# gau-nernst/centernet-lightning

Hardware: AMD Instinct MI355X
Metric: images/sec @512x512 ResNet34 CenterNet forward + gather_detection2d (higher is better)
Workload: dtype f32; 1 GPU; BASELINE C1: ResNet34 + simple neck, 32 img/GPU x 512x512, heads 80+4 (w256), k=100, nms 3; global_batch=32, per_gpu_batch=32, parallelism=batch-shard x1

## Files before the change

### centernet-lightning_amd/centernet_lightning_amd/_lib.py

```python
import ctypes
import os
from ctypes import (POINTER, Structure, c_char_p, c_double, c_float, c_int32, c_int64, c_size_t, c_uint32, c_void_p)

_LIB_NAME = "libcenternet_gfx950.so"
_LIB_PATH = os.path.join(os.path.dirname(os.path.abspath(__file__)), "lib", _LIB_NAME)

CNL_RELU = 1 << 0
CNL_SIGMOID = 1 << 1
CNL_UPSAMPLE_IN = 1 << 2
CNL_UPSAMPLE_OUT_ADD = 1 << 3
CNL_RELU6 = 1 << 4
CNL_W_SPLIT = 1 << 5

CNL_ALGO_AUTO, CNL_ALGO_F2, CNL_ALGO_F32, CNL_ALGO_LATENCY, CNL_ALGO_F43, CNL_ALGO_FORCE = 0, 1, 2, 4, 5, 100
CNL_WINO_F32, CNL_WINO_F16X2 = 2, 5

CNL_E_BAD_ARG, CNL_E_UNSUPPORTED, CNL_E_WORKSPACE, CNL_E_HIP = -1, -2, -3, -4
ABI_VERSION = 13


class ConvParams(Structure):
    _fields_ = [("x", c_void_p), ("w", c_void_p), ("bias", c_void_p), ("residual", c_void_p), ("y", c_void_p),
                ("N", c_int32), ("H_in", c_int32), ("W_in", c_int32), ("Cin", c_int32), ("Cout", c_int32),
                ("KH", c_int32), ("KW", c_int32), ("stride", c_int32), ("pad", c_int32),
# ... 44 lines not shown


class MotTables(Structure):
    POINTERS = ("gt_boxes", "pr_boxes", "gt_ids", "pr_ids", "gt_off", "pr_off", "sim_off", "frm_seq", "seq_frm", "seq_gid", "seq_tid", "seq_pair",
                "seq_idm", "gt_count", "pr_count")
    SCALARS = ("F", "S", "n_gt", "n_pr", "sim_total", "pair_total", "sum_g", "sum_t", "id_total", "max_gids", "max_gt_frame", "max_pr_frame",
               "max_frame_pairs")
    _fields_ = [(n, c_void_p) for n in POINTERS] + [(n, c_int64) for n in SCALARS]


class LossParams(Structure):
    _fields_ = [("stride", c_double), ("target_param", c_double), ("hm_alpha", c_double), ("hm_beta", c_double),
                ("heatmap_weight", c_double), ("box_weight", c_double), ("box_multiplier", c_float), ("target_method", c_int32),
                ("heatmap_loss", c_int32), ("box_loss", c_int32), ("box_log", c_int32), ("reserved", c_int32)]


class ReidLossParams(Structure):
    _fields_ = [("stride", c_double), ("bn_eps", c_double), ("momentum", c_double), ("ignore_index", c_int64), ("center", c_int32),
                ("padded_rows", c_int32), ("training", c_int32), ("reserved", c_int32)]


class AugmentPlacement(Structure):
    _fields_ = [("frame", c_int32), ("x0", c_int32), ("y0", c_int32), ("w", c_int32), ("h", c_int32), ("dx0", c_int32), ("dy0", c_int32),
                ("dw", c_int32), ("dh", c_int32), ("flip", c_int32), ("colour", c_int32 * 12), ("reserved", c_int32 * 2)]


class WarpPlacement(Structure):
    _fields_ = [("frame", c_int32), ("x0", c_int32), ("y0", c_int32), ("w", c_int32), ("h", c_int32), ("dx0", c_int32), ("dy0", c_int32),
                ("dw", c_int32), ("dh", c_int32), ("reserved0", c_int32), ("colour", c_int32 * 12), ("inv", c_int64 * 6), ("fwd", c_double * 6),
                ("reserved", c_int32 * 2)]


assert ctypes.sizeof(LetterboxFrame) == 40 and ctypes.sizeof(AugmentPlacement) == 96 and ctypes.sizeof(WarpPlacement) == 192

_REID_COMMON = [c_void_p, c_int64, c_int64, c_int64, c_int64, c_int32, c_int32, c_int32, c_int32, c_void_p, c_void_p, c_void_p, c_int32,
                c_void_p, c_void_p, c_void_p, c_void_p, c_void_p, c_void_p, c_void_p, c_int32, POINTER(ReidLossParams)]

_SIGNATURES = {
    "cnl_version": (ctypes.c_int, []),
    "cnl_sizeof_params": (c_size_t, [ctypes.c_int32]),
    "cnl_absmax_stride": (ctypes.c_int, []),
    "cnl_last_error": (c_size_t, [c_char_p, c_size_t]),
    "cnl_conv2d_nhwc_f32": (ctypes.c_int, [POINTER(ConvParams), c_void_p]),
    "cnl_fused_out_pack_weights_f32": (ctypes.c_int, [c_void_p, c_void_p, ctypes.c_int32, ctypes.c_int32, c_void_p]),
    "cnl_fused_out_reduce_f32": (ctypes.c_int, [c_void_p, ctypes.c_int32, ctypes.c_int64, ctypes.c_int32, c_void_p, c_void_p, ctypes.c_int32, ctypes.c_uint32, c_void_p]),
    "cnl_pointwise_nhwc_f32": (ctypes.c_int, [POINTER(ConvParams), c_void_p, c_int32, c_int32, c_int32, c_int32, c_int32, c_void_p, c_void_p]),
    "cnl_conv2d_out_hw": (ctypes.c_int, [POINTER(ConvParams), POINTER(c_int32), POINTER(c_int32)]),
    "cnl_conv3x3_winograd_f32": (ctypes.c_int, [POINTER(ConvParams), c_void_p]),
    "cnl_conv3x3_winograd_kernel": (ctypes.c_int, [POINTER(ConvParams)]),
    "cnl_winograd_up_weight_floats": (c_size_t, [ctypes.c_int32, ctypes.c_int32]),
    "cnl_winograd_transform_weights_up_f32": (ctypes.c_int, [c_void_p, c_void_p, ctypes.c_int32, ctypes.c_int32, c_void_p]),
    "cnl_conv3x3_winograd_variant": (ctypes.c_int, [POINTER(ConvParams)]),
    "cnl_conv2d_kernel": (ctypes.c_int, [POINTER(ConvParams)]),
    "cnl_up2_weight_floats": (c_size_t, [ctypes.c_int32, ctypes.c_int32]),
    "cnl_up2_pack_weights_f32": (ctypes.c_int, [c_void_p, c_void_p, ctypes.c_int32, ctypes.c_int32, c_void_p]),
    "cnl_conv3x3_up2_nhwc_f32": (ctypes.c_int, [POINTER(ConvParams), c_void_p]),
    "cnl_conv3x3_up2_kernel": (ctypes.c_int, [POINTER(ConvParams)]),
    "cnl_absmax_per_image_f32": (ctypes.c_int, [c_void_p, ctypes.c_int32, ctypes.c_int64, ctypes.c_int32, ctypes.c_int32, c_void_p, c_void_p]),
    "cnl_winograd_weight_floats": (c_size_t, [c_int32, c_int32]),
    "cnl_winograd_transform_weights_f32": (ctypes.c_int, [c_void_p, c_void_p, c_int32, c_int32, c_void_p]),
    "cnl_deconv2x_nhwc_f32": (ctypes.c_int, [POINTER(DeconvParams), c_void_p]),
    "cnl_deconv_phase_geometry": (ctypes.c_int, [c_int32, c_int32, POINTER(c_int32), POINTER(c_int32)]),
    "cnl_deconv_weight_floats": (c_size_t, [c_int32, c_int32, c_int32]),
    "cnl_conv2d_splitk_scratch_bytes": (c_size_t, [POINTER(ConvParams)]),
    "cnl_fuse_sum_nhwc_f32": (ctypes.c_int, [c_void_p, c_void_p, c_void_p, c_void_p, c_int32, c_int32, c_int32, c_int32, c_int32, c_int32,
                                             c_int32, c_int32, ctypes.c_float, ctypes.c_float, ctypes.c_float, ctypes.c_float, c_int32, c_void_p]),
    "cnl_upsample2x_nhwc_f32": (ctypes.c_int, [c_void_p, c_void_p, c_void_p, c_int32, c_int32, c_int32, c_int32, c_int32, c_int32,
                                               c_int32, c_int32, c_void_p]),
    "cnl_depthwise3x3_nhwc_f32": (ctypes.c_int, [c_void_p, c_void_p, c_void_p, c_void_p, c_int32, c_int32, c_int32, c_int32, c_int32,
                                                 c_int32, c_uint32, c_void_p]),
    "cnl_deform_sample_nhwc_f32": (ctypes.c_int, [c_void_p, c_void_p, c_void_p, c_int32, c_int32, c_int32, c_int32, c_int32, c_int32,
                                                  c_int32, c_int32, c_void_p]),
    "cnl_normalize_u8_nhwc_f32": (ctypes.c_int, [c_void_p, c_void_p, c_int32, c_int32, c_int32, POINTER(c_float), POINTER(c_float), c_void_p]),
    "cnl_resize_bilinear_u8": (ctypes.c_int, [c_void_p, c_void_p, c_int32, c_int32, c_int32, c_int32, c_int32, c_int32, c_void_p]),
    "cnl_letterbox_bilinear_u8": (ctypes.c_int, [c_void_p, c_void_p, c_int32, c_int32, c_int32, c_int32, c_uint32, c_void_p]),
    "cnl_letterbox_yuv420_u8": (ctypes.c_int, [c_void_p, c_void_p, c_int32, c_int32, c_int32, POINTER(c_int32), c_uint32, c_void_p]),
    "cnl_unletterbox_boxes_f32": (ctypes.c_int, [c_void_p, c_void_p, c_int32, c_int32, c_int32, c_void_p]),
    "cnl_crop_boxes_u8": (ctypes.c_int, [c_void_p, c_void_p, c_void_p, c_float, c_void_p, c_int32, c_int32, c_int32, POINTER(c_int32), c_float,
                                         c_int32, c_void_p, c_void_p, c_void_p, c_int32, c_int32, c_uint32, c_void_p]),
    "cnl_draw_boxes_u8": (ctypes.c_int, [c_void_p, c_void_p, c_void_p, c_void_p, c_void_p, c_float, c_void_p, c_int32, c_int32, c_int32, c_int32,
                                         c_void_p, c_int32, c_int32, c_int32, c_int32, c_int32, c_int32, c_void_p, c_void_p]),
    "cnl_flip_merge_f32": (ctypes.c_int, [POINTER(FlipMap), c_int32, c_int32, c_int32, c_int32, c_void_p]),
    "cnl_mirror_append_u8": (ctypes.c_int, [c_void_p, c_void_p, c_int32, c_int32, c_int32, c_int32, c_void_p]),
    "cnl_merge_tiles_workspace_bytes": (c_size_t, [c_int32, c_int32, c_int32, c_int32]),
    "cnl_merge_tiles_f32": (ctypes.c_int, [c_void_p, c_void_p, c_void_p, c_void_p, c_void_p, c_int32, c_int32, c_int32, c_int32, c_int32,
                                           c_float, c_float, c_int32, c_int32, c_void_p, c_void_p, c_void_p, c_void_p, c_void_p, c_void_p,
                                           c_size_t, c_void_p]),
    "cnl_coco_match_f64": (ctypes.c_int, [c_void_p, c_void_p, c_void_p, c_void_p, c_void_p, c_void_p, c_void_p, c_int32, c_int32, c_int32, c_int32,
                                          c_void_p, c_void_p, c_void_p, c_void_p, c_void_p]),
    "cnl_coco_accumulate_f64": (ctypes.c_int, [c_void_p, c_void_p, c_void_p, c_void_p, c_void_p, c_int64, c_int32, c_void_p, c_void_p, c_void_p]),
    "cnl_mot_similarity_f64": (ctypes.c_int, [POINTER(MotTables), c_void_p, c_void_p]),
    "cnl_mot_hota_workspace_bytes": (c_int64, [POINTER(MotTables)]),
    "cnl_mot_hota_f64": (ctypes.c_int, [POINTER(MotTables), c_void_p, c_void_p, c_void_p, c_void_p, c_void_p, c_void_p, c_int64, c_void_p]),
    "cnl_mot_clear_workspace_bytes": (c_int64, [POINTER(MotTables)]),
    "cnl_mot_clear_f64": (ctypes.c_int, [POINTER(MotTables), c_void_p, c_void_p, c_void_p, c_void_p, c_void_p, c_int64, c_void_p]),
    "cnl_mot_identity_workspace_bytes": (c_int64, [POINTER(MotTables)]),
    "cnl_mot_identity_f64": (ctypes.c_int, [POINTER(MotTables), c_void_p, c_void_p, c_void_p, c_void_p, c_void_p, c_int64, c_void_p]),
    "cnl_detection_loss_workspace_bytes": (c_size_t, [c_int32, c_int32, c_int32, c_int32]),
    "cnl_detection_loss_f64": (ctypes.c_int, [c_void_p, c_int64, c_int64, c_int64, c_int64, c_void_p, c_int64, c_int64, c_int64, c_int64,
                                              c_int32, c_int32, c_int32, c_int32, c_void_p, c_void_p, c_void_p, c_int32, POINTER(LossParams),
                                              c_void_p, c_int64, c_int64, c_int64, c_int64, c_void_p, c_void_p, c_void_p, c_void_p, c_size_t,
                                              c_void_p]),
    "cnl_detection_loss_grad_workspace_bytes": (c_size_t, [c_int32, c_int32, c_int32, c_int32]),
    "cnl_detection_loss_grad_f32": (ctypes.c_int, [c_void_p, c_int64, c_int64, c_int64, c_int64, c_void_p, c_int64, c_int64, c_int64, c_int64,
                                                   c_int32, c_int32, c_int32, c_int32, c_void_p, c_void_p, c_void_p, c_int32, POINTER(LossParams),
                                                   c_void_p, c_void_p, c_int64, c_int64, c_int64, c_int64, c_void_p, c_int64, c_int64, c_int64,
# ... 135 lines not shown
```

### centernet-lightning_amd/csrc/conv_args.h

```cpp
#pragma once
#include "cnl_device.h"

namespace cnl_conv {
using namespace cnl_dev;


struct ConvArgs {
    const float* x;
    const float* w;
    const float* bias;
    const float* res;
    float* y;
    int N, Hin, Win, Cin, Cout;
    int KH, KW, stride, pad, pad_x;
    int sub_dy, sub_dx;
    int ldx, ldy, ldr;
    int HL, WL;
    int Ho, Wo, M;
    int CC, KT, K;
    unsigned x_bytes, w_bytes, y_bytes, r_bytes;
    unsigned flags;
    int tiles_n, tiles;
    unsigned mg_hw, sh_hw, mg_w, sh_w;
    long long* trace;
    const float* xmax;
    const float* wmax;
    unsigned* ymax;
    unsigned algo;
    const float* wscale;
    const float* wsplit = nullptr;
    int ksplit = 0, kt_per = 0;
    float* part = nullptr;
    unsigned part_bytes = 0;
};

constexpr unsigned CNL_I_SUBPIXEL = 1u << 16;

template <int WM, int WN, int TM, int TN>
struct Cfg {
    static constexpr int NW = WM * WN;
    static constexpr int THREADS = NW * 64;
    static constexpr int BM = WM * TM * 32;
    static constexpr int BN = WN * TN * 32;
    static constexpr int A_INSTR = BM / (NW * 8);
    static constexpr int B_INSTR = BN / (NW * 8);
    static constexpr int STAGE_BYTES = (BM + BN) * 128;
    static constexpr int LDS_BYTES = 2 * STAGE_BYTES;
    static_assert(NW == 4, "kernel is declared __launch_bounds__(256, 2)");
    static_assert(BM % (NW * 8) == 0 && BN % (NW * 8) == 0, "tile rows must split evenly over waves");
};


__device__ __forceinline__ f32x4 buf_load4(const float* base, unsigned bytes, unsigned voffset, unsigned soffset) {
    const auto rsrc = __builtin_amdgcn_make_buffer_rsrc((void*)base, 0, (int)bytes, 0x00020000);
    return __builtin_bit_cast(f32x4, __builtin_amdgcn_raw_buffer_load_b128(rsrc, voffset, soffset, 0));
}
__device__ __forceinline__ void buf_store4(f32x4 v, float* base, unsigned bytes, unsigned voffset, unsigned soffset) {
    typedef unsigned u32x4_ __attribute__((ext_vector_type(4)));
    const auto rsrc = __builtin_amdgcn_make_buffer_rsrc((void*)base, 0, (int)bytes, 0x00020000);
    __builtin_amdgcn_raw_buffer_store_b128(__builtin_bit_cast(u32x4_, v), rsrc, voffset, soffset, CNL_NT_STORES);
}
__device__ __forceinline__ f32x4 lds_read16(const char* p) { return *reinterpret_cast<const f32x4*>(p); }
__device__ __forceinline__ unsigned fast_div(unsigned n, unsigned magic, unsigned shift) {
    return shift == 0xFFu ? n : (__umulhi(n, magic) >> shift);
}


bool f16x2_eligible(const ConvArgs& a);
int f16x2_launch(const ConvArgs& a, hipStream_t stream);

}
```

### centernet-lightning_amd/csrc/conv_f16x2.hip

```cpp
#include "conv_args.h"
#include <cstdlib>

namespace cnl_conv {



template <int WM, int WN, int TM, int TN, int KS, bool SUB, bool SPLIT = false, bool PREB = false>
__global__ __launch_bounds__(256, 2) void conv_f16x2_kernel(const ConvArgs a) {
    using C = Cfg<WM, WN, TM, TN>;
    constexpr bool PRE = SUB || PREB;
    extern __shared__ __attribute__((aligned(16))) char smem[];
    float* sInv = reinterpret_cast<float*>(smem + C::LDS_BYTES);
    float* sScl = sInv + C::BM;
    int* sImg = reinterpret_cast<int*>(sScl + C::BM);
    unsigned* sPix = reinterpret_cast<unsigned*>(sImg + C::BM);

    const int lane = threadIdx.x & 63;
    const int wave = __builtin_amdgcn_readfirstlane(threadIdx.x >> 6);
    const int wm = wave / WN, wn = wave % WN;
    const int hi = lane >> 5;

    unsigned tile = cnl::xcd_remap(blockIdx.x, (unsigned)a.tiles);
    int slice = 0;
    if constexpr (SPLIT) { slice = (int)(tile % (unsigned)a.ksplit); tile /= (unsigned)a.ksplit; }
    const int kt0 = SPLIT ? slice * a.kt_per : 0;
    const int KTs = SPLIT ? min(a.kt_per, a.KT - kt0) : a.KT;
    const int n_tile = tile % a.tiles_n;
    const int m_tile = tile / a.tiles_n;
    const int m0 = m_tile * C::BM;
    const int n0 = n_tile * C::BN;

    const int lrow = lane >> 3;
    const int pslot = lane & 7;
    unsigned a_mask[C::A_INSTR], a_base[C::A_INSTR];
#pragma unroll
    for (int j = 0; j < C::A_INSTR; ++j) {
        const int r = (j * C::NW + wave) * 8 + lrow;
        const int m = m0 + r;
        const int q = (pslot ^ ((r >> 1) & 7)) * 4;
        const unsigned n = fast_div((unsigned)m, a.mg_hw, a.sh_hw);
        const unsigned rem = (unsigned)m - n * (unsigned)(a.Ho * a.Wo);
        const unsigned oy = fast_div(rem, a.mg_w, a.sh_w);
        const unsigned ox = rem - oy * (unsigned)a.Wo;
        const int iy0 = (int)oy * a.stride - a.pad;
        const int ix0 = (int)ox * a.stride - a.pad_x;
        unsigned mask = 0, xb = 0;
#pragma unroll
        for (int kx = 0; kx < KS; ++kx) xb |= ((unsigned)(ix0 + kx) < (unsigned)a.WL) ? (1u << kx) : 0u;
#pragma unroll
        for (int ky = 0; ky < KS; ++ky) mask |= ((unsigned)(iy0 + ky) < (unsigned)a.HL) ? (xb << (ky * KS)) : 0u;
        a_mask[j] = m < a.M ? mask : 0u;
        const int pix = (int)n * a.Hin * a.Win;
        a_base[j] = (unsigned)(((pix + iy0 * a.Win + ix0) * a.ldx + q) * 4);
    }
    unsigned b_off[C::B_INSTR];
#pragma unroll
    for (int j = 0; j < C::B_INSTR; ++j) {
        const int r = (j * C::NW + wave) * 8 + lrow;
        const int q = (pslot ^ ((r >> 1) & 7)) * 4;
        b_off[j] = (unsigned)(((n0 + r) * a.K + q) * 4);
    }
    unsigned a_voff[C::A_INSTR];
#define C5_TAP(tap_, ky_, kx_)                                                                                    \
    do {                                                                                                          \
        const unsigned bit_ = 1u << (tap_);                                                                       \
        const unsigned delta_ = (unsigned)((((ky_) * a.Win + (kx_)) * a.ldx) * 4);                                \
        _Pragma("unroll") for (int j = 0; j < C::A_INSTR; ++j) a_voff[j] = (a_mask[j] & bit_) ? a_base[j] + delta_ : OOB; \
    } while (0)
// ... 36 lines not shown
            const unsigned oy = fast_div(rem, a.mg_w, a.sh_w);
            const unsigned ox = rem - oy * (unsigned)a.Wo;
            sPix[r] = (n * 2u * (unsigned)a.Ho + 2u * oy + (unsigned)a.sub_dy) * (2u * (unsigned)a.Wo) + 2u * ox + (unsigned)a.sub_dx;
        }
    }

    f32x16 acc[TM][TN];
#pragma unroll
    for (int i = 0; i < TM; ++i)
#pragma unroll
        for (int j = 0; j < TN; ++j) acc[i][j] = mfma_zero();

    const int swz = (lane >> 1) & 7;
    const int a_row_byte = (wm * TM * 32 + (lane & 31)) * 128;
    const int b_row_byte = C::BM * 128 + (wn * TN * 32 + (lane & 31)) * 128;
    f32x4 ra[2][TM], rb[2][TN];
    u32x4 ah[TM], al[TM], bh[TN], bl[TN];
    float sA[TM];

#define C5_READ(stage_ptr_, g_)                                                                                   \
    do {                                                                                                          \
        _Pragma("unroll") for (int q_ = 0; q_ < 2; ++q_) {                                                        \
            const int sb_ = (((2 * (2 * (g_) + q_) + hi) ^ swz) << 4);                                            \
               \
            const int sbb_ = PRE ? (((2 * (2 * (g_) + hi) + q_) ^ swz) << 4) : sb_;                               \
            _Pragma("unroll") for (int i = 0; i < TM; ++i) ra[q_][i] = lds_read16((stage_ptr_) + a_row_byte + i * 32 * 128 + sb_); \
            _Pragma("unroll") for (int j = 0; j < TN; ++j) rb[q_][j] = lds_read16((stage_ptr_) + b_row_byte + j * 32 * 128 + sbb_); \
        }                                                                                                         \
    } while (0)
#define C5_SPLIT()                                                                                                \
    do {                                                                                                          \
        _Pragma("unroll") for (int i = 0; i < TM; ++i) split8(ra[0][i], ra[1][i], sA[i], ah[i], al[i]);           \
        _Pragma("unroll") for (int j = 0; j < TN; ++j) {                                                          \
            if constexpr (PRE) {                                                                                  \
                bh[j] = __builtin_bit_cast(u32x4, rb[0][j]);                                                      \
                bl[j] = __builtin_bit_cast(u32x4, rb[1][j]);                                                      \
            } else {                                                                                              \
                split8(rb[0][j], rb[1][j], Sw, bh[j], bl[j]);                                                     \
            }                                                                                                     \
        }                                                                                                         \
    } while (0)
#define C5_MFMA()                                                                                                 \
    do {                                                                                                          \
        _Pragma("unroll") for (int i = 0; i < TM; ++i)                                                            \
            _Pragma("unroll") for (int j = 0; j < TN; ++j) acc[i][j] = mfma16(ah[i], bl[j], acc[i][j]);           \
        _Pragma("unroll") for (int i = 0; i < TM; ++i)                                                            \
            _Pragma("unroll") for (int j = 0; j < TN; ++j) acc[i][j] = mfma16(al[i], bh[j], acc[i][j]);           \
        _Pragma("unroll") for (int i = 0; i < TM; ++i)                                                            \
            _Pragma("unroll") for (int j = 0; j < TN; ++j) acc[i][j] = mfma16(ah[i], bh[j], acc[i][j]);           \
    } while (0)

    asm volatile("s_waitcnt vmcnt(0)" ::: "memory");
    __syncthreads();
#pragma unroll
    for (int i = 0; i < TM; ++i) sA[i] = sScl[(wm * TM + i) * 32 + (lane & 31)];
    if (KTs > 1) {
        C5_ADVANCE();
        C5_ISSUE(1, cc * 32, (kt0 + 1) * 32);
    }
    C5_READ(smem, 0);
    for (int kt = 0; kt < KTs; ++kt) {
        const char* sS = smem + (kt & 1) * C::STAGE_BYTES;
        const char* sN = smem + ((kt + 1) & 1) * C::STAGE_BYTES;
        C5_SPLIT();
        C5_READ(sS, 1);
        C5_MFMA();
        C5_SPLIT();
        if (kt + 1 < KTs) {
            asm volatile("s_waitcnt vmcnt(0)" ::: "memory");
            __syncthreads();
            if (kt + 2 < KTs) {
                C5_ADVANCE();
                C5_ISSUE(kt & 1, cc * 32, (kt0 + kt + 2) * 32);
            }
            C5_READ(sN, 0);
        }
        C5_MFMA();
    }
#undef C5_TAP
#undef C5_ISSUE
#undef C5_ADVANCE
#undef C5_READ
#undef C5_SPLIT
#undef C5_MFMA

    if constexpr (SPLIT) {
#pragma unroll
        for (int j = 0; j < TN; ++j) {
            const int col = n0 + (wn * TN + j) * 32 + (lane & 31);
#pragma unroll
            for (int i = 0; i < TM; ++i) {
                const int rl = (wm * TM + i) * 32 + 4 * hi;
                const int mb = m0 + rl;
#pragma unroll
                for (int r = 0; r < 16; ++r) {
                    const int ro = (r & 3) + 8 * (r >> 2);
                    const bool ok = col < a.Cout && mb + ro < a.M;
                    buf_store(acc[i][j][r] * sInv[rl + ro], a.part, a.part_bytes,
                              ok ? (unsigned)((((long long)slice * a.M + mb + ro) * a.Cout + col) * 4) : OOB, 0u);
                }
            }
        }
        return;
    }
    const float lo = (a.flags & (CNL_RELU | CNL_RELU6)) ? 0.f : -__builtin_inff();
    const float hi6 = (a.flags & CNL_RELU6) ? 6.f : __builtin_inff();
    const bool sigm = a.flags & CNL_SIGMOID;
    const int img0 = sImg[0];
    float omax = 0.f, omax1 = 0.f;
#pragma unroll
    for (int j = 0; j < TN; ++j) {
        const int col = n0 + (wn * TN + j) * 32 + (lane & 31);
        const bool col_ok = col < a.Cout;
        const float bv = col_ok ? a.bias[col] : 0.f;
#pragma unroll
        for (int i = 0; i < TM; ++i) {
            const int rl = (wm * TM + i) * 32 + 4 * hi;
            const int mb = m0 + rl;
            const unsigned y_voff = (unsigned)((mb * a.ldy + col) * 4);
            const unsigned r_voff = (unsigned)((mb * a.ldr + col) * 4);
            float v[16];
            bool ok[16];
#pragma unroll
            for (int r = 0; r < 16; ++r) {
                const int ro = (r & 3) + 8 * (r >> 2);
                ok[r] = col_ok && mb + ro < a.M;
                v[r] = acc[i][j][r] * sInv[rl + ro] + bv;
            }
            if (!SUB && a.res) {
                float rv[16];
#pragma unroll
                for (int r = 0; r < 16; ++r)
                    rv[r] = buf_load(a.res, a.r_bytes, ok[r] ? r_voff : OOB, (unsigned)(((r & 3) + 8 * (r >> 2)) * a.ldr * 4));
#pragma unroll
                for (int r = 0; r < 16; ++r) v[r] += rv[r];
            }
#pragma unroll
            for (int r = 0; r < 16; ++r) v[r] = fminf(fmaxf(v[r], lo), hi6);
            if (sigm) {
#pragma unroll
                for (int r = 0; r < 16; ++r) v[r] = cnl::fast_sigmoid(v[r]);
            }
            if constexpr (SUB) {
#pragma unroll
                for (int r = 0; r < 16; ++r)
                    buf_store(v[r], a.y, a.y_bytes, ok[r] ? (sPix[rl + (r & 3) + 8 * (r >> 2)] * (unsigned)a.ldy + (unsigned)col) * 4u : OOB, 0u);
            } else {
#pragma unroll
                for (int r = 0; r < 16; ++r)
                    buf_store(v[r], a.y, a.y_bytes, ok[r] ? y_voff : OOB, (unsigned)(((r & 3) + 8 * (r >> 2)) * a.ldy * 4));
            }
            if (a.ymax) {
#pragma unroll
                for (int r = 0; r < 16; ++r) {
                    const float av = ok[r] ? fabsf(v[r]) : 0.f;
                    const int img = sImg[rl + (r & 3) + 8 * (r >> 2)];
                    if (img == img0) omax = fmaxf(omax, av);
                    else if (img == img0 + 1) omax1 = fmaxf(omax1, av);
                    else if (av > 0.f) cnl::report_max(a.ymax + img * AMS, av);
                }
            }
        }
    }
    if (a.ymax) {
#pragma unroll
        for (int o = 32; o > 0; o >>= 1) {
            omax = fmaxf(omax, __shfl_xor(omax, o, 64));
            omax1 = fmaxf(omax1, __shfl_xor(omax1, o, 64));
        }
        if (lane == 0) cnl::report_max(a.ymax + img0 * AMS, omax);
        if (lane == 0) cnl::report_max(a.ymax + (img0 + 1) * AMS, omax1);
    }
}

__global__ __launch_bounds__(256) void splitk_reduce_kernel(const ConvArgs a) {
    const int C4 = (a.Cout + 3) / 4;
    const long total = (long)a.M * C4;
    const long t = (long)blockIdx.x * 256 + threadIdx.x;
    float omax = 0.f;
    int img = -1;
    if (t < total) {
        const int m = (int)(t / C4), col = (int)(t - (long)m * C4) * 4;
        img = (int)fast_div((unsigned)m, a.mg_hw, a.sh_hw);
        const bool vec = col + 4 <= a.Cout && (a.Cout & 3) == 0;
        float v[4] = {0.f, 0.f, 0.f, 0.f};
        const long sstride = (long)a.M * a.Cout;
        const float* p0 = a.part + (long)m * a.Cout + col;
        if (vec) {
            for (int s0 = 0; s0 < a.ksplit; s0 += 8) {
                f32x4 q[8];
#pragma unroll
                for (int j = 0; j < 8; ++j)
                    q[j] = s0 + j < a.ksplit ? *reinterpret_cast<const f32x4*>(p0 + (s0 + j) * sstride) : f32x4{0.f, 0.f, 0.f, 0.f};
#pragma unroll
                for (int j = 0; j < 8; ++j)
#pragma unroll
                    for (int i = 0; i < 4; ++i) v[i] += q[j][i];
            }
        } else {
            for (int s = 0; s < a.ksplit; ++s)
#pragma unroll
                for (int i = 0; i < 4; ++i)
                    if (col + i < a.Cout) v[i] += p0[s * sstride + i];
        }
        const float lo = (a.flags & (CNL_RELU | CNL_RELU6)) ? 0.f : -__builtin_inff();
        const float hi6 = (a.flags & CNL_RELU6) ? 6.f : __builtin_inff();
#pragma unroll
        for (int i = 0; i < 4; ++i) {
            if (col + i >= a.Cout) continue;
            float o = v[i] + a.bias[col + i];
            if (a.res) o += a.res[(long)m * a.ldr + col + i];
            o = fminf(fmaxf(o, lo), hi6);
            if (a.flags & CNL_SIGMOID) o = cnl::fast_sigmoid(o);
            a.y[(long)m * a.ldy + col + i] = o;
            omax = fmaxf(omax, fabsf(o));
        }
    }
    if (a.ymax) {
        const int img0 = __shfl(img, 0, 64);
        const bool same = __all(img == img0 || img < 0);
        if (same) {
#pragma unroll
            for (int o = 32; o > 0; o >>= 1) omax = fmaxf(omax, __shfl_xor(omax, o, 64));
            if ((threadIdx.x & 63) == 0 && img0 >= 0) cnl::report_max(a.ymax + img0 * AMS, omax);
        } else if (img >= 0 && omax > 0.f) {
            atomicMax(a.ymax + img * AMS, __float_as_uint(omax));
        }
    }
}

template <int KS>
static int launch_split5(const ConvArgs& in, hipStream_t stream) {
    using C = Cfg<2, 2, 1, 2>;
    ConvArgs a = in;
    const int tiles_m = (a.M + C::BM - 1) / C::BM;
    a.tiles_n = (a.Cout + C::BN - 1) / C::BN;
    a.tiles = tiles_m * a.tiles_n * a.ksplit;
    static cnl::DeviceOnce once;
    int rc = cnl::kernel_setup(once, reinterpret_cast<const void*>(&conv_f16x2_kernel<2, 2, 1, 2, KS, false, true>), 160 * 1024);
    if (rc != CNL_OK) return rc;
    hipLaunchKernelGGL((conv_f16x2_kernel<2, 2, 1, 2, KS, false, true>), dim3(a.tiles), dim3(C::THREADS), C::LDS_BYTES + C::BM * 16, stream, a);
    rc = cnl::check_launch("conv_f16x2_kernel (split)");
    if (rc != CNL_OK) return rc;
    const long total = (long)a.M * ((a.Cout + 3) / 4);
    hipLaunchKernelGGL(splitk_reduce_kernel, dim3((unsigned)((total + 255) / 256)), dim3(256), 0, stream, a);
    return cnl::check_launch("splitk_reduce_kernel");
}

template <int WM, int WN, int TM, int TN, int KS, bool SUB, bool PREB = false>
static int launch_one5(const ConvArgs& a, hipStream_t stream) {
    using C = Cfg<WM, WN, TM, TN>;
    static cnl::DeviceOnce once;
    const int rc = cnl::kernel_setup(once, reinterpret_cast<const void*>(&conv_f16x2_kernel<WM, WN, TM, TN, KS, SUB, false, PREB>), 160 * 1024);
    if (rc != CNL_OK) return rc;
    hipLaunchKernelGGL((conv_f16x2_kernel<WM, WN, TM, TN, KS, SUB, false, PREB>), dim3(a.tiles), dim3(C::THREADS), C::LDS_BYTES + C::BM * 16, stream, a);
    return cnl::check_launch("conv_f16x2_kernel");
}

template <int WM, int WN, int TM, int TN>
static int launch_cfg5(const ConvArgs& in, hipStream_t stream) {
    using C = Cfg<WM, WN, TM, TN>;
    ConvArgs a = in;
    const int tiles_m = (a.M + C::BM - 1) / C::BM;
    a.tiles_n = (a.Cout + C::BN - 1) / C::BN;
    a.tiles = tiles_m * a.tiles_n;
    if (a.flags & CNL_I_SUBPIXEL) return launch_one5<WM, WN, TM, TN, 2, true>(a, stream);
    if (a.wsplit) return a.KH == 3 ? launch_one5<WM, WN, TM, TN, 3, false, true>(a, stream) : launch_one5<WM, WN, TM, TN, 1, false, true>(a, stream);
    return a.KH == 3 ? launch_one5<WM, WN, TM, TN, 3, false>(a, stream) : launch_one5<WM, WN, TM, TN, 1, false>(a, stream);
}

bool f16x2_eligible(const ConvArgs& a) {
    const long long min_out_1x1 = a.algo == CNL_ALGO_FORCE + 5 ? 0 : (1ll << 20);
    if (a.algo == CNL_ALGO_F32 || !a.xmax || (a.flags & (CNL_UPSAMPLE_IN | CNL_UPSAMPLE_OUT_ADD))) return false;
    if (a.flags & CNL_I_SUBPIXEL) return a.KH == 2 && a.KW == 2 && !a.res && a.wscale;
    return (a.wmax || (a.wsplit && a.ksplit <= 1)) && a.KH == a.KW && (a.KH == 1 || a.KH == 3) && a.pad == a.pad_x &&
           (a.KH == 3 || a.ksplit > 1 || (long long)a.Ho * a.Wo * a.Cout >= min_out_1x1);
}

int f16x2_launch(const ConvArgs& a, hipStream_t s) {
    if (a.ksplit > 1 && !(a.flags & CNL_I_SUBPIXEL)) return a.KH == 3 ? launch_split5<3>(a, s) : launch_split5<1>(a, s);
    if (a.Cout <= 32) return launch_cfg5<4, 1, 2, 1>(a, s);
    if (a.Cout <= 64) return launch_cfg5<4, 1, 2, 2>(a, s);
    if (a.Cout <= 96) return launch_cfg5<4, 1, 1, 3>(a, s);
    const long long tiles128 = (((long long)a.M + 127) / 128) * ((a.Cout + 127) / 128);
    if (tiles128 < 512) return launch_cfg5<2, 2, 1, 2>(a, s);
    return launch_cfg5<4, 1, 1, 4>(a, s);
}

}
```

### centernet-lightning_amd/csrc/conv_mfma.hip

```cpp
#include "conv_args.h"
#include <cstdlib>

namespace cnl_conv {

__device__ __forceinline__ f32x16 mfma32(float a, float b, f32x16 c) {
    return __builtin_amdgcn_mfma_f32_32x32x2f32(a, b, c, 0, 0, 0);
}
__device__ __forceinline__ f32x16 mfma_zero() {
    const f32x16 z = {0.f, 0.f, 0.f, 0.f, 0.f, 0.f, 0.f, 0.f, 0.f, 0.f, 0.f, 0.f, 0.f, 0.f, 0.f, 0.f};
    return __builtin_amdgcn_mfma_f32_32x32x2f32(0.f, 0.f, z, 0, 0, 0);
}
template <bool CHECK, bool RES>
__device__ __forceinline__ void store_tile(const f32x16& acc, float bv, float lo, float hi6, bool sigm, const ConvArgs& a, unsigned y_voff,
                                           unsigned r_voff, int m_base, bool col_ok) {
    float v[16];
    if constexpr (RES) {
        float rv[16];
#pragma unroll
        for (int r = 0; r < 16; ++r) {
            const int ro = (r & 3) + 8 * (r >> 2);
            const bool ok = !CHECK || (col_ok && m_base + ro < a.M);
            rv[r] = buf_load(a.res, a.r_bytes, ok ? r_voff : OOB, (unsigned)(ro * a.ldr * 4));
        }
#pragma unroll
// ... 452 lines not shown
    if (f16x2_eligible(a)) {
        if (a.ksplit > 1) {
            const int per = (a.KT + a.ksplit - 1) / a.ksplit;
            const unsigned long long pb = (unsigned long long)a.ksplit * (unsigned long long)M * a.Cout * 4ull;
            if (per >= 2 && !out4x && !(a.flags & CNL_UPSAMPLE_IN) && pb < lim) {
                a.kt_per = per;
                a.ksplit = (a.KT + per - 1) / per;
                a.part_bytes = (unsigned)((unsigned long long)a.ksplit * (unsigned long long)M * a.Cout * 4ull);
            } else {
                a.ksplit = 0;
            }
        }
        return f16x2_launch(a, s);
    }
    a.ksplit = 0;
    if (a.Cout <= 32) return launch_cfg<4, 1, 2, 1>(a, s);
    if (a.Cout <= 64) return launch_cfg<4, 1, 2, 2>(a, s);
    if (a.Cout <= 96) return launch_cfg<4, 1, 1, 3>(a, s);
    const long long tiles128 = ((M + 127) / 128) * ((a.Cout + 127) / 128);
    if (tiles128 < 512) return launch_cfg<2, 2, 1, 2>(a, s);
    return launch_cfg<2, 2, 2, 2>(a, s);
}

extern "C" int cnl_conv2d_out_hw(const cnl_conv_params* p, int32_t* H_out, int32_t* W_out) {
    CNL_REQUIRE(p && H_out && W_out, CNL_E_BAD_ARG, "cnl_conv2d_out_hw: null argument");
    CNL_REQUIRE(p->stride > 0 && p->KH > 0 && p->KW > 0, CNL_E_BAD_ARG, "cnl_conv2d_out_hw: bad kernel/stride");
    const int up = (p->flags & CNL_UPSAMPLE_IN) ? 2 : 1;
    *H_out = (p->H_in * up + 2 * p->pad - p->KH) / p->stride + 1;
    *W_out = (p->W_in * up + 2 * p->pad - p->KW) / p->stride + 1;
    return CNL_OK;
}

extern "C" size_t cnl_conv2d_splitk_scratch_bytes(const cnl_conv_params* p) {
    if (!p || p->splitk <= 1) return 0;
    int32_t ho = 0, wo = 0;
    if (cnl_conv2d_out_hw(p, &ho, &wo) != CNL_OK || ho <= 0 || wo <= 0) return 0;
    return (size_t)p->splitk * (size_t)p->N * (size_t)ho * (size_t)wo * (size_t)p->Cout * 4;
}

extern "C" int cnl_conv2d_kernel(const cnl_conv_params* p) {
    CNL_REQUIRE(p, CNL_E_BAD_ARG, "cnl_conv2d_kernel: null params");
    ConvArgs a;
    a.KH = p->KH; a.KW = p->KW; a.pad = a.pad_x = p->pad; a.flags = p->flags; a.Cout = p->Cout;
    a.xmax = p->x_absmax; a.wmax = p->w_absmax; a.wscale = nullptr; a.res = p->residual; a.algo = p->algo;
    a.wsplit = (p->flags & CNL_W_SPLIT) ? p->w : nullptr;
    a.ksplit = p->splitk > 1 ? p->splitk : 0;
    int32_t ho = 0, wo = 0;
    const int rc = cnl_conv2d_out_hw(p, &ho, &wo);
    if (rc != CNL_OK) return rc;
    a.Ho = ho; a.Wo = wo;
    return f16x2_eligible(a) ? CNL_CONV_F16X2 : CNL_CONV_F32;
}

extern "C" int cnl_conv2d_nhwc_f32(const cnl_conv_params* p, void* stream) {
    CNL_REQUIRE(p, CNL_E_BAD_ARG, "cnl_conv2d_nhwc_f32: null params");
    CNL_REQUIRE(p->x && p->w && p->bias && p->y, CNL_E_BAD_ARG, "cnl_conv2d_nhwc_f32: null tensor pointer");
    CNL_REQUIRE(p->N > 0 && p->H_in > 0 && p->W_in > 0 && p->Cin > 0 && p->Cout > 0, CNL_E_BAD_ARG,
                "cnl_conv2d_nhwc_f32: non-positive dimension");
    CNL_REQUIRE(p->KH > 0 && p->KW > 0 && p->stride > 0 && p->pad >= 0, CNL_E_BAD_ARG,
                "cnl_conv2d_nhwc_f32: bad kernel/stride/pad");
    CNL_REQUIRE(p->KH * p->KW <= 32, CNL_E_UNSUPPORTED, "cnl_conv2d_nhwc_f32: KH*KW = %d > 32 taps", p->KH * p->KW);
    CNL_REQUIRE(p->Cin % 32 == 0, CNL_E_UNSUPPORTED,
                "cnl_conv2d_nhwc_f32: Cin=%d is not a multiple of 32 (use cnl_stem_conv7x7_f32 for the RGB stem)", p->Cin);
    CNL_REQUIRE(p->ldx >= p->Cin && p->ldy >= p->Cout && p->ldx % 4 == 0, CNL_E_BAD_ARG,
                "cnl_conv2d_nhwc_f32: pixel strides ldx=%d ldy=%d too small / misaligned", p->ldx, p->ldy);
    CNL_REQUIRE(((uintptr_t)p->x & 15) == 0 && ((uintptr_t)p->w & 15) == 0, CNL_E_BAD_ARG,
                "cnl_conv2d_nhwc_f32: x and w must be 16-byte aligned");
    const bool up_out = p->flags & CNL_UPSAMPLE_OUT_ADD;
    CNL_REQUIRE(!up_out || p->residual, CNL_E_BAD_ARG, "cnl_conv2d_nhwc_f32: CNL_UPSAMPLE_OUT_ADD needs a residual");
    CNL_REQUIRE(!up_out || !(p->flags & CNL_SIGMOID), CNL_E_UNSUPPORTED, "cnl_conv2d_nhwc_f32: sigmoid with UPSAMPLE_OUT_ADD");
    CNL_REQUIRE(!p->residual || p->ldr >= p->Cout, CNL_E_BAD_ARG, "cnl_conv2d_nhwc_f32: ldr=%d < Cout", p->ldr);

    ConvArgs a;
    a.x = p->x; a.w = p->w; a.bias = p->bias; a.res = p->residual; a.y = p->y;
    a.N = p->N; a.Hin = p->H_in; a.Win = p->W_in; a.Cin = p->Cin; a.Cout = p->Cout;
    a.KH = p->KH; a.KW = p->KW; a.stride = p->stride; a.pad = a.pad_x = p->pad;
    a.sub_dy = a.sub_dx = 0;
    a.ldx = p->ldx; a.ldy = p->ldy; a.ldr = p->ldr;
    a.flags = p->flags;
    a.xmax = p->x_absmax; a.wmax = p->w_absmax; a.ymax = reinterpret_cast<unsigned*>(p->y_absmax); a.wscale = nullptr; a.algo = p->algo;
    if (p->flags & CNL_W_SPLIT) {
        CNL_REQUIRE(p->KH == p->KW && (p->KH == 1 || p->KH == 3), CNL_E_BAD_ARG, "cnl_conv2d_nhwc_f32: CNL_W_SPLIT with a %d x %d kernel", p->KH, p->KW);
        const size_t total = (size_t)p->Cout * p->KH * p->KW * p->Cin;
        a.wsplit = p->w + total;
        a.wscale = p->w + 2 * total;
    }
    const int up = (p->flags & CNL_UPSAMPLE_IN) ? 2 : 1;
    a.HL = p->H_in * up; a.WL = p->W_in * up;
    a.Ho = (a.HL + 2 * p->pad - p->KH) / p->stride + 1;
    a.Wo = (a.WL + 2 * p->pad - p->KW) / p->stride + 1;
    if (p->splitk > 1) {
        CNL_REQUIRE(p->splitk <= 256, CNL_E_BAD_ARG, "cnl_conv2d_nhwc_f32: splitk=%d (at most 256 slices)", p->splitk);
        CNL_REQUIRE(p->splitk_scratch && ((uintptr_t)p->splitk_scratch & 15) == 0 && p->splitk_scratch_bytes >= cnl_conv2d_splitk_scratch_bytes(p),
                    CNL_E_WORKSPACE, "cnl_conv2d_nhwc_f32: splitk_scratch missing, unaligned or smaller than cnl_conv2d_splitk_scratch_bytes()");
        a.ksplit = p->splitk;
        a.part = p->splitk_scratch;
    }
    return finish_and_launch(a, up_out, "cnl_conv2d_nhwc_f32", (hipStream_t)stream);
}

namespace cnl_conv {
__global__ __launch_bounds__(256) void up2_pack_kernel(const float* __restrict__ w, float* __restrict__ wp, int Cin, int Cout) {
    const long total = 16l * Cin * Cout;
    for (long e = (long)blockIdx.x * 256 + threadIdx.x; e < total; e += (long)gridDim.x * 256) {
        const int ci = (int)(e % Cin);
        long t = e / Cin;
// ... 191 lines not shown
```

### include/centernet_gfx950.h

```cpp
#ifndef CENTERNET_GFX950_H
#define CENTERNET_GFX950_H

#include <stddef.h>
#include <stdint.h>

#ifdef __cplusplus
extern "C" {
#endif
#if defined(__GNUC__) || defined(__clang__)
#pragma GCC visibility push(default)
#endif

#define CNL_ABI_VERSION 13

enum {
    CNL_OK = 0,
    CNL_E_BAD_ARG = -1,
    CNL_E_UNSUPPORTED = -2,
    CNL_E_WORKSPACE = -3,
    CNL_E_HIP = -4
};

enum {
    CNL_ALGO_AUTO = 0,
    CNL_ALGO_F2 = 1,
    CNL_ALGO_F32 = 2,
    CNL_ALGO_LATENCY = 4,
    CNL_ALGO_F43 = 5,
    CNL_ALGO_FORCE = 100
};

enum {
    CNL_RELU = 1u << 0,
    CNL_SIGMOID = 1u << 1,
    CNL_UPSAMPLE_IN = 1u << 2,
    CNL_UPSAMPLE_OUT_ADD = 1u << 3,
    CNL_RELU6 = 1u << 4,
    CNL_W_SPLIT = 1u << 5
};

typedef struct cnl_conv_params {
    const float* x;
    const float* w;
    const float* bias;
    const float* residual;
    float* y;
    int32_t N, H_in, W_in, Cin, Cout;
    int32_t KH, KW, stride, pad;
    int32_t ldx, ldy, ldr;
    uint32_t flags;
    const float* x_absmax;
    float* y_absmax;
    const float* w_absmax;
    uint32_t algo;
    int32_t splitk;
    float* splitk_scratch;
    size_t splitk_scratch_bytes;
    const float* fuse_w;
    float* fuse_part;
    const float* w_up;
} cnl_conv_params;

int cnl_fused_out_pack_weights_f32(const float* w_ohwi, float* fuse_w, int32_t Cout, int32_t C2, void* stream);
int cnl_fused_out_reduce_f32(const float* part, int32_t nblocks, int64_t M, int32_t C2, const float* bias, float* y, int32_t ldy,
                             uint32_t flags, void* stream);
int cnl_conv2d_nhwc_f32(const cnl_conv_params* p, void* stream);
size_t cnl_winograd_up_weight_floats(int32_t Cin, int32_t Cout);
int cnl_winograd_transform_weights_up_f32(const float* w_ohwi, float* u_up, int32_t Cin, int32_t Cout, void* stream);
size_t cnl_conv2d_splitk_scratch_bytes(const cnl_conv_params* p);

#define CNL_CONV_F32 2
#define CNL_CONV_F16X2 5
int cnl_conv2d_kernel(const cnl_conv_params* p);

size_t cnl_conv_split_weight_floats(int32_t Cin, int32_t Cout, int32_t KH, int32_t KW);
int cnl_conv_split_weights_f32(const float* w_ohwi, float* w_buf, int32_t Cin, int32_t Cout, int32_t KH, int32_t KW, void* stream);
int cnl_pointwise_nhwc_f32(const cnl_conv_params* p, const float* x2, int32_t H2, int32_t W2, int32_t C2, int32_t ldx2, int32_t stride2,
                           const float* x2_absmax, void* stream);
size_t cnl_up2_weight_floats(int32_t Cin, int32_t Cout);
int cnl_up2_pack_weights_f32(const float* w_ohwi, float* w_packed, int32_t Cin, int32_t Cout, void* stream);
int cnl_conv3x3_up2_nhwc_f32(const cnl_conv_params* p, void* stream);
int cnl_conv3x3_up2_kernel(const cnl_conv_params* p);

int cnl_absmax_stride(void);
int cnl_absmax_per_image_f32(const float* x, int32_t N, int64_t pixels, int32_t C, int32_t ld, float* out, void* stream);

int cnl_conv2d_out_hw(const cnl_conv_params* p, int32_t* H_out, int32_t* W_out);

#define CNL_WINO_F32 2
#define CNL_WINO_BF16X3 3
#define CNL_WINO_F16X2 5
int cnl_conv3x3_winograd_f32(const cnl_conv_params* p, void* stream);
int cnl_conv3x3_winograd_kernel(const cnl_conv_params* p);
int cnl_conv3x3_winograd_variant(const cnl_conv_params* p);
size_t cnl_winograd_weight_floats(int32_t Cin, int32_t Cout);
int cnl_winograd_transform_weights_f32(const float* w_ohwi, float* u, int32_t Cin, int32_t Cout, void* stream);
int cnl_normalize_u8_nhwc_f32(const uint8_t* x, float* y, int32_t N, int32_t H, int32_t W, const float* mean255,
                              const float* inv_std255, void* stream);

int cnl_resize_bilinear_u8(const uint8_t* x, uint8_t* y, int32_t N, int32_t H_in, int32_t W_in, int32_t H_out, int32_t W_out,
                           int32_t C, void* stream);

typedef struct cnl_letterbox_frame {
    const void* src;
    int32_t h, w;
    int32_t row_stride;
    int32_t new_h, new_w;
    int32_t pad_top, pad_left;
    int32_t reserved;
} cnl_letterbox_frame;
int cnl_letterbox_bilinear_u8(const void* table, uint8_t* out, int32_t N, int32_t height, int32_t width, int32_t C,
                              uint32_t fill_rgba, void* stream);

int cnl_unletterbox_boxes_f32(float* boxes, const void* table, int32_t N, int32_t k, int32_t clip, void* stream);

typedef struct cnl_yuv420_frame {
    const void* y;
    const void* u;
    const void* v;
    int32_t y_pitch, c_pitch;
    int32_t c_step;
    int32_t x0, y0;
    int32_t h, w;
    int32_t new_h, new_w;
    int32_t pad_top, pad_left;
    int32_t reserved;
// ... 266 lines not shown
```

Before: 4244 images/s.

## Add persistent streaming f16x2 kernel for small 1x1 convolutions

Adds a persistent 512-thread kernel for 1x1 stride-1 convs with Cout<=96 and K<=256. It keeps the whole split weight matrix resident in LDS and streams 32-row activation blocks through a four-deep register ring, prefetching the next row block while computing the current one. The aim is to cut per-tile launch and LDS staging overhead for the head/neck pointwise convs. It also adds a form query API and optional cycle-trace instrumentation compiled out by default. The cost is high register pressure and an untested new epilogue path.

```diff
diff --git a/centernet-lightning_amd/centernet_lightning_amd/_lib.py b/centernet-lightning_amd/centernet_lightning_amd/_lib.py
--- a/centernet-lightning_amd/centernet_lightning_amd/_lib.py
+++ b/centernet-lightning_amd/centernet_lightning_amd/_lib.py
@@ -120,6 +120,7 @@
     "cnl_winograd_transform_weights_up_f32": (ctypes.c_int, [c_void_p, c_void_p, ctypes.c_int32, ctypes.c_int32, c_void_p]),
     "cnl_conv3x3_winograd_variant": (ctypes.c_int, [POINTER(ConvParams)]),
     "cnl_conv2d_kernel": (ctypes.c_int, [POINTER(ConvParams)]),
+    "cnl_conv2d_form": (ctypes.c_int, [POINTER(ConvParams)]),
     "cnl_up2_weight_floats": (c_size_t, [ctypes.c_int32, ctypes.c_int32]),
     "cnl_up2_pack_weights_f32": (ctypes.c_int, [c_void_p, c_void_p, ctypes.c_int32, ctypes.c_int32, c_void_p]),
     "cnl_conv3x3_up2_nhwc_f32": (ctypes.c_int, [POINTER(ConvParams), c_void_p]),
diff --git a/centernet-lightning_amd/csrc/conv_args.h b/centernet-lightning_amd/csrc/conv_args.h
--- a/centernet-lightning_amd/csrc/conv_args.h
+++ b/centernet-lightning_amd/csrc/conv_args.h
@@ -67,6 +67,7 @@
 
 
 bool f16x2_eligible(const ConvArgs& a);
+bool f16x2_streams(const ConvArgs& a);
 int f16x2_launch(const ConvArgs& a, hipStream_t stream);
 
 }
diff --git a/centernet-lightning_amd/csrc/conv_f16x2.hip b/centernet-lightning_amd/csrc/conv_f16x2.hip
--- a/centernet-lightning_amd/csrc/conv_f16x2.hip
+++ b/centernet-lightning_amd/csrc/conv_f16x2.hip
@@ -1,9 +1,13 @@
 #include "conv_args.h"
 #include <cstdlib>
 
+#ifdef C5_TRACE
+#define C5_TRACE_ROWS 81
+static long long* g_c5_trace = nullptr;
+extern "C" __attribute__((visibility("default"))) void cnl_c5_set_trace(void* p) { g_c5_trace = (long long*)p; }
+#endif
+
 namespace cnl_conv {
-
-
 
 template <int WM, int WN, int TM, int TN, int KS, bool SUB, bool SPLIT = false, bool PREB = false>
 __global__ __launch_bounds__(256, 2) void conv_f16x2_kernel(const ConvArgs a) {
@@ -14,6 +18,15 @@
     float* sScl = sInv + C::BM;
     int* sImg = reinterpret_cast<int*>(sScl + C::BM);
     unsigned* sPix = reinterpret_cast<unsigned*>(sImg + C::BM);
+#ifdef C5_TRACE
+    unsigned long long* trl = reinterpret_cast<unsigned long long*>(smem + C::LDS_BYTES + C::BM * 16);
+    const bool tr_on = a.trace && blockIdx.x == 0 && threadIdx.x == 0;
+#define C5_STAMP(row_, i_) do { if (tr_on && (row_) < C5_TRACE_ROWS) trl[(row_) * 8 + (i_)] = __builtin_readcyclecounter(); } while (0)
+    if (tr_on) for (int i = 0; i < C5_TRACE_ROWS * 8; ++i) trl[i] = 0ull;
+#else
+#define C5_STAMP(row_, i_) do {} while (0)
+#endif
+    C5_STAMP(0, 0);
 
     const int lane = threadIdx.x & 63;
     const int wave = __builtin_amdgcn_readfirstlane(threadIdx.x >> 6);
@@ -156,6 +169,7 @@
 
     asm volatile("s_waitcnt vmcnt(0)" ::: "memory");
     __syncthreads();
+    C5_STAMP(0, 1);
 #pragma unroll
     for (int i = 0; i < TM; ++i) sA[i] = sScl[(wm * TM + i) * 32 + (lane & 31)];
     if (KTs > 1) {
@@ -166,21 +180,30 @@
     for (int kt = 0; kt < KTs; ++kt) {
         const char* sS = smem + (kt & 1) * C::STAGE_BYTES;
         const char* sN = smem + ((kt + 1) & 1) * C::STAGE_BYTES;
+        C5_STAMP(1 + kt, 0);
         C5_SPLIT();
         C5_READ(sS, 1);
+        C5_STAMP(1 + kt, 1);
         C5_MFMA();
+        C5_STAMP(1 + kt, 2);
         C5_SPLIT();
+        C5_STAMP(1 + kt, 3);
         if (kt + 1 < KTs) {
             asm volatile("s_waitcnt vmcnt(0)" ::: "memory");
+            C5_STAMP(1 + kt, 4);
             __syncthreads();
+            C5_STAMP(1 + kt, 5);
             if (kt + 2 < KTs) {
                 C5_ADVANCE();
                 C5_ISSUE(kt & 1, cc * 32, (kt0 + kt + 2) * 32);
             }
             C5_READ(sN, 0);
+            C5_STAMP(1 + kt, 6);
         }
         C5_MFMA();
-    }
+        C5_STAMP(1 + kt, 7);
+    }
+    C5_STAMP(0, 2);
 #undef C5_TAP
 #undef C5_ISSUE
 #undef C5_ADVANCE
@@ -275,6 +298,14 @@
         if (lane == 0) cnl::report_max(a.ymax + img0 * AMS, omax);
         if (lane == 0) cnl::report_max(a.ymax + (img0 + 1) * AMS, omax1);
     }
+#ifdef C5_TRACE
+    if (tr_on) {
+        asm volatile("s_waitcnt vmcnt(0)" ::: "memory");
+        C5_STAMP(0, 3);
+        for (int i = 0; i < C5_TRACE_ROWS * 8; ++i) a.trace[i] = (long long)trl[i];
+    }
+#endif
+#undef C5_STAMP
 }
 
 __global__ __launch_bounds__(256) void splitk_reduce_kernel(const ConvArgs a) {
@@ -333,6 +364,177 @@
     }
 }
 
+template <int TN, bool FULL>
+__global__ __launch_bounds__(512, 2) void conv_f16x2_stream_kernel(const ConvArgs a) {
+    constexpr int BN = TN * 32, D = 4;
+    extern __shared__ __attribute__((aligned(16))) char smem[];
+    const int lane = threadIdx.x & 63;
+    const int wave = __builtin_amdgcn_readfirstlane(threadIdx.x >> 6);
+    const int hi = lane >> 5, l31 = lane & 31;
+    const int KT = a.KT, KTp = (KT + D - 1) & ~(D - 1);
+    const int RB = a.tiles;
+    {
+        const int lrow = lane >> 3, pslot = lane & 7;
+        const int pieces = KT * (BN / 8);
+        for (int p = wave; p < pieces; p += 8) {
+            const int kt = p / (BN / 8);
+            const int r = (p - kt * (BN / 8)) * 8 + lrow;
+            const int q = (pslot ^ ((r >> 1) & 7)) * 4;
+            dma16(a.wsplit, a.w_bytes, smem + p * 1024, (unsigned)((r * a.K + q) * 4), (unsigned)(kt * 128));
+        }
+    }
+    const float Sw = *a.wscale;
+    const int rb_step = (int)gridDim.x * 8;
+    int rb = (int)blockIdx.x * 8 + wave;
+    auto row_of = [&](int rb_) { return min(rb_ * 32 + l31, a.M - 1); };
+    int m_cur = row_of(min(rb, RB - 1));
+    unsigned voff_cur = (unsigned)m_cur * (unsigned)a.ldx * 4u + (unsigned)hi * 16u;
+    unsigned n_cur = fast_div((unsigned)m_cur, a.mg_hw, a.sh_hw);
+    float mx_cur = a.xmax[n_cur * AMS];
+
+    f32x4 ring[D][4];
+#define C5S_LOAD(s_, voff_, kt_)                                                                                  \
+    do {                                                                                                          \
+        _Pragma("unroll") for (int f_ = 0; f_ < 4; ++f_)                                                          \
+            ring[s_][f_] = __builtin_bit_cast(f32x4, buf_load16(a.x, a.x_bytes, (voff_), (unsigned)((kt_) * 128 + f_ * 32))); \
+    } while (0)
+#pragma unroll
+    for (int s = 0; s < D; ++s) C5S_LOAD(s, voff_cur, min(s, KT - 1));
+
+    const int swz = (lane >> 1) & 7;
+    f32x16 acc[TN];
+    float bias_j[TN];
+#pragma unroll
+    for (int j = 0; j < TN; ++j) bias_j[j] = j * 32 + l31 < a.Cout ? a.bias[j * 32 + l31] : 0.f;
+    asm volatile("s_waitcnt vmcnt(0)" ::: "memory");
+    __syncthreads();
+    while (rb < RB) {
+        const int rb_n = rb + rb_step;
+        const int m_nxt = row_of(min(rb_n, RB - 1));
+        const unsigned voff_nxt = (unsigned)m_nxt * (unsigned)a.ldx * 4u + (unsigned)hi * 16u;
+        const unsigned n_nxt = fast_div((unsigned)m_nxt, a.mg_hw, a.sh_hw);
+        const float mx_nxt = a.xmax[n_nxt * AMS];
+        const float S = pow2_scale(mx_cur);
+        const int img0 = __builtin_amdgcn_readfirstlane((int)n_cur);
+        const unsigned seen0 = a.ymax ? cnl::peek_max(a.ymax + img0 * AMS) : 0u;
+#pragma unroll
+        for (int j = 0; j < TN; ++j) acc[j] = mfma_zero();
+        for (int kt0 = 0; kt0 < KTp; kt0 += D) {
+#pragma unroll
+            for (int s = 0; s < D; ++s) {
+                const int kt = kt0 + s;
+                const bool live = FULL || kt < KT;
+                u32x4 ah[2], al[2];
+                if (live) {
+#pragma unroll
+                    for (int g = 0; g < 2; ++g) split8(ring[s][2 * g], ring[s][2 * g + 1], S, ah[g], al[g]);
+                }
+                __builtin_amdgcn_sched_barrier(0);
+                const bool wrap = kt + D >= KTp;
+                const int ktn = wrap ? s : kt + D;
+                C5S_LOAD(s, wrap ? voff_nxt : voff_cur, min(ktn, KT - 1));
+                __builtin_amdgcn_sched_barrier(0);
+                if (live) {
+                    const char* sBk = smem + kt * (BN * 128) + l31 * 128;
+#pragma unroll
+                    for (int g = 0; g < 2; ++g) {
+                        u32x4 bh[TN], bl[TN];
+#pragma unroll
+                        for (int j = 0; j < TN; ++j) {
+                            bh[j] = lds_u4(sBk + j * 32 * 128 + (((2 * (2 * g + hi)) ^ swz) << 4));
+                            bl[j] = lds_u4(sBk + j * 32 * 128 + (((2 * (2 * g + hi) + 1) ^ swz) << 4));
+                        }
+#pragma unroll
+                        for (int j = 0; j < TN; ++j) acc[j] = mfma16(ah[g], bl[j], acc[j]);
+#pragma unroll
+                        for (int j = 0; j < TN; ++j) acc[j] = mfma16(al[g], bh[j], acc[j]);
+#pragma unroll
+                        for (int j = 0; j < TN; ++j) acc[j] = mfma16(ah[g], bh[j], acc[j]);
+                    }
+                }
+            }
+        }
+        const int m0 = rb * 32;
+        const float inv = 1.f / (S * Sw);
+        const int img = (int)n_cur;
+        const int rl = 4 * hi;
+        const float lo = (a.flags & (CNL_RELU | CNL_RELU6)) ? 0.f : -__builtin_inff();
+        const float hi6 = (a.flags & CNL_RELU6) ? 6.f : __builtin_inff();
+        const bool sigm = a.flags & CNL_SIGMOID;
+        float omax = 0.f, omax1 = 0.f;
+        const int mb = m0 + rl;
+#pragma unroll
+        for (int j = 0; j < TN; ++j) {
+            const int col = j * 32 + l31;
+            const bool col_ok = col < a.Cout;
+            const float bv = bias_j[j];
+            const unsigned y_voff = (unsigned)((mb * a.ldy + col) * 4);
+            const unsigned r_voff = (unsigned)((mb * a.ldr + col) * 4);
+            float v[16];
+            bool ok[16];
+#pragma unroll
+            for (int r = 0; r < 16; ++r) {
+                const int ro = (r & 3) + 8 * (r >> 2);
+                ok[r] = col_ok && mb + ro < a.M;
+                v[r] = acc[j][r] * __shfl(inv, rl + ro, 64) + bv;
+            }
+            if (a.res) {
+                float rv[16];
+#pragma unroll
+                for (int r = 0; r < 16; ++r)
+                    rv[r] = buf_load(a.res, a.r_bytes, ok[r] ? r_voff : OOB, (unsigned)(((r & 3) + 8 * (r >> 2)) * a.ldr * 4));
+#pragma unroll
+                for (int r = 0; r < 16; ++r) v[r] += rv[r];
+            }
+#pragma unroll
+            for (int r = 0; r < 16; ++r) v[r] = fminf(fmaxf(v[r], lo), hi6);
+            if (sigm) {
+#pragma unroll
+                for (int r = 0; r < 16; ++r) v[r] = cnl::fast_sigmoid(v[r]);
+            }
+#pragma unroll
+            for (int r = 0; r < 16; ++r)
+                buf_store(v[r], a.y, a.y_bytes, ok[r] ? y_voff : OOB, (unsigned)(((r & 3) + 8 * (r >> 2)) * a.ldy * 4));
+            if (a.ymax) {
+#pragma unroll
+                for (int r = 0; r < 16; ++r) {
+                    const float av = ok[r] ? fabsf(v[r]) : 0.f;
+                    const int img_r = __shfl(img, rl + (r & 3) + 8 * (r >> 2), 64);
+                    if (img_r == img0) omax = fmaxf(omax, av);
+                    else if (img_r == img0 + 1) omax1 = fmaxf(omax1, av);
+                    else if (av > 0.f) cnl::report_max(a.ymax + img_r * AMS, av);
+                }
+            }
+        }
+        if (a.ymax) {
+            omax = cnl::wave_max_nonneg(omax);
+            omax1 = cnl::wave_max_nonneg(omax1);
+            if (lane == 0) cnl::raise_max(a.ymax + img0 * AMS, omax, seen0);
+            if (lane == 0) cnl::report_max(a.ymax + (img0 + 1) * AMS, omax1);
+        }
+        rb = rb_n; voff_cur = voff_nxt; n_cur = n_nxt; mx_cur = mx_nxt;
+    }
+#undef C5S_LOAD
+}
+
+template <int TN, bool FULL>
+static int launch_stream5_one(const ConvArgs& a, hipStream_t stream) {
+    static cnl::DeviceOnce once;
+    int n_cu = 0;
+    const int rc = cnl::kernel_setup(once, reinterpret_cast<const void*>(&conv_f16x2_stream_kernel<TN, FULL>), 160 * 1024, &n_cu);
+    if (rc != CNL_OK) return rc;
+    hipLaunchKernelGGL((conv_f16x2_stream_kernel<TN, FULL>), dim3(min(n_cu, (a.tiles + 7) / 8)), dim3(512), a.KT * TN * 32 * 128, stream, a);
+    return cnl::check_launch("conv_f16x2_stream_kernel");
+}
+
+template <int TN>
+static int launch_stream5(const ConvArgs& in, hipStream_t stream) {
+    ConvArgs a = in;
+    a.tiles_n = 1;
+    a.tiles = (a.M + 31) / 32;
+    return a.KT % 4 == 0 ? launch_stream5_one<TN, true>(a, stream) : launch_stream5_one<TN, false>(a, stream);
+}
+
 template <int KS>
 static int launch_split5(const ConvArgs& in, hipStream_t stream) {
     using C = Cfg<2, 2, 1, 2>;
@@ -357,7 +559,13 @@
     static cnl::DeviceOnce once;
     const int rc = cnl::kernel_setup(once, reinterpret_cast<const void*>(&conv_f16x2_kernel<WM, WN, TM, TN, KS, SUB, false, PREB>), 160 * 1024);
     if (rc != CNL_OK) return rc;
+#ifdef C5_TRACE
+    ConvArgs t = a;
+    t.trace = g_c5_trace;
+    hipLaunchKernelGGL((conv_f16x2_kernel<WM, WN, TM, TN, KS, SUB, false, PREB>), dim3(a.tiles), dim3(C::THREADS), C::LDS_BYTES + C::BM * 16 + C5_TRACE_ROWS * 64, stream, t);
+#else
     hipLaunchKernelGGL((conv_f16x2_kernel<WM, WN, TM, TN, KS, SUB, false, PREB>), dim3(a.tiles), dim3(C::THREADS), C::LDS_BYTES + C::BM * 16, stream, a);
+#endif
     return cnl::check_launch("conv_f16x2_kernel");
 }
 
@@ -374,15 +582,21 @@
 }
 
 bool f16x2_eligible(const ConvArgs& a) {
-    const long long min_out_1x1 = a.algo == CNL_ALGO_FORCE + 5 ? 0 : (1ll << 20);
+    const long long min_out_1x1 = (a.algo == CNL_ALGO_FORCE + 5 || a.algo == CNL_ALGO_FORCE + 15) ? 0 : (1ll << 20);
     if (a.algo == CNL_ALGO_F32 || !a.xmax || (a.flags & (CNL_UPSAMPLE_IN | CNL_UPSAMPLE_OUT_ADD))) return false;
     if (a.flags & CNL_I_SUBPIXEL) return a.KH == 2 && a.KW == 2 && !a.res && a.wscale;
     return (a.wmax || (a.wsplit && a.ksplit <= 1)) && a.KH == a.KW && (a.KH == 1 || a.KH == 3) && a.pad == a.pad_x &&
            (a.KH == 3 || a.ksplit > 1 || (long long)a.Ho * a.Wo * a.Cout >= min_out_1x1);
 }
 
+bool f16x2_streams(const ConvArgs& a) {
+    return a.algo != CNL_ALGO_FORCE + 15 && a.wsplit && a.ksplit <= 1 && !(a.flags & CNL_I_SUBPIXEL) && a.KH == 1 && a.KW == 1 && a.stride == 1 &&
+           a.pad == 0 && a.Cout <= 96 && a.K <= 256;
+}
+
 int f16x2_launch(const ConvArgs& a, hipStream_t s) {
     if (a.ksplit > 1 && !(a.flags & CNL_I_SUBPIXEL)) return a.KH == 3 ? launch_split5<3>(a, s) : launch_split5<1>(a, s);
+    if (f16x2_streams(a)) return a.Cout <= 32 ? launch_stream5<1>(a, s) : a.Cout <= 64 ? launch_stream5<2>(a, s) : launch_stream5<3>(a, s);
     if (a.Cout <= 32) return launch_cfg5<4, 1, 2, 1>(a, s);
     if (a.Cout <= 64) return launch_cfg5<4, 1, 2, 2>(a, s);
     if (a.Cout <= 96) return launch_cfg5<4, 1, 1, 3>(a, s);
diff --git a/centernet-lightning_amd/csrc/conv_mfma.hip b/centernet-lightning_amd/csrc/conv_mfma.hip
--- a/centernet-lightning_amd/csrc/conv_mfma.hip
+++ b/centernet-lightning_amd/csrc/conv_mfma.hip
@@ -528,6 +528,19 @@
     return f16x2_eligible(a) ? CNL_CONV_F16X2 : CNL_CONV_F32;
 }
 
+extern "C" int cnl_conv2d_form(const cnl_conv_params* p) {
+    CNL_REQUIRE(p, CNL_E_BAD_ARG, "cnl_conv2d_form: null params");
+    const int k = cnl_conv2d_kernel(p);
+    if (k != CNL_CONV_F16X2) return k < 0 ? k : CNL_CONV_FORM_TILE;
+    ConvArgs a;
+    a.KH = p->KH; a.KW = p->KW; a.stride = p->stride; a.pad = a.pad_x = p->pad; a.flags = p->flags; a.Cout = p->Cout; a.algo = p->algo;
+    a.K = p->KH * p->KW * p->Cin;
+    a.wsplit = (p->flags & CNL_W_SPLIT) ? p->w : nullptr;
+    a.ksplit = p->splitk > 1 ? p->splitk : 0;
+    if (a.ksplit > 1 && (a.K / 32 + a.ksplit - 1) / a.ksplit < 2) a.ksplit = 0;
+    return f16x2_streams(a) ? CNL_CONV_FORM_STREAM : CNL_CONV_FORM_TILE;
+}
+
 extern "C" int cnl_conv2d_nhwc_f32(const cnl_conv_params* p, void* stream) {
     CNL_REQUIRE(p, CNL_E_BAD_ARG, "cnl_conv2d_nhwc_f32: null params");
     CNL_REQUIRE(p->x && p->w && p->bias && p->y, CNL_E_BAD_ARG, "cnl_conv2d_nhwc_f32: null tensor pointer");
diff --git a/include/centernet_gfx950.h b/include/centernet_gfx950.h
--- a/include/centernet_gfx950.h
+++ b/include/centernet_gfx950.h
@@ -72,6 +72,9 @@
 #define CNL_CONV_F32 2
 #define CNL_CONV_F16X2 5
 int cnl_conv2d_kernel(const cnl_conv_params* p);
+#define CNL_CONV_FORM_TILE 0
+#define CNL_CONV_FORM_STREAM 1
+int cnl_conv2d_form(const cnl_conv_params* p);
 
 size_t cnl_conv_split_weight_floats(int32_t Cin, int32_t Cout, int32_t KH, int32_t KW);
 int cnl_conv_split_weights_f32(const float* w_ohwi, float* w_buf, int32_t Cin, int32_t Cout, int32_t KH, int32_t KW, void* stream);
```

New measurement: 4251 images/s (median of 6 runs). Within noise of the previous version (+0.2%).
